# Gregor-Mendel-Institute/SNPmatch

Measured on AMD Instinct MI355X. Metric: accession×SNP comparisons/sec (whole node); achieved HBM GB/s vs peak, higher is better.
Workload: dtype f64

## Files before the change

snpmatch_amd/csrc/snpm_api_launch.hpp:

```cpp
struct FastGeom {
    bool packed;
    int wpb;
    int tile_rows = TILE_ROWS;
    int64_t n_wc, n_colblocks, n_parts, part_rows;
    int64_t n_epochs, n_slots, n_groups;
};

template <bool SKIP, bool GATHER>
int occupancy_of(int threads)
{
    int nb = 0;
    if (hipOccupancyMaxActiveBlocksPerMultiprocessor(&nb, k_fast<SKIP, GATHER>, threads, 0) != hipSuccess) nb = 0;
    return nb;
}

FastGeom fast_geom(snpm_ctx *ctx, int64_t n_acc, int64_t n, int occ_blocks_hint, bool packed, int tile_rows = TILE_ROWS,
                   int wpb_fixed = 0, int kernel_parts_mult = 1)
{
    FastGeom g;
    g.packed = packed;
    g.tile_rows = tile_rows;
    const int64_t span = (int64_t)WAVE * (packed ? 16 : 4);
    g.n_wc = std::max<int64_t>(1, (n_acc + span - 1) / span);
    if (wpb_fixed > 0) {
        g.wpb = (int)std::min<int64_t>(wpb_fixed, g.n_wc);
    } else if (g.n_wc <= 8) {
        g.wpb = (int)g.n_wc;
    } else {
        double best = -1.0;
        int best_w = 8;
        for (int w = 8; w >= 4; --w) {
            const int64_t blocks = (g.n_wc + w - 1) / w;
            const double active = (double)g.n_wc / (double)(blocks * w);
            const double balance = (w % 4 == 0) ? 1.0 : ((w % 2 == 0) ? 0.95 : 0.85);
            if (active * balance > best) { best = active * balance; best_w = w; }
        }
        g.wpb = best_w;
    }
    g.n_colblocks = (g.n_wc + g.wpb - 1) / g.wpb;
    int occ = occ_blocks_hint > 0 ? occ_blocks_hint : 2;
    const int64_t pitch_bytes = ((n_acc + 255) / 256) * 256;
    if (!packed && occ_blocks_hint > 0 && (g.wpb == 4 || g.wpb == 5) &&
        n * pitch_bytes >= (int64_t(32) << 30))
        occ = std::min(occ, std::max(3, 18 / g.wpb));
    if (!packed && occ_blocks_hint > 0 && g.wpb == 8 &&
        n * pitch_bytes >= (int64_t(4) << 30))
        occ = std::min(occ, 2);
    const int narrow_mult = (!packed && g.wpb == 1 && occ_blocks_hint > 0) ? 4 : 1;
    const int64_t n_tiles = std::max<int64_t>(1, (n + tile_rows - 1) / tile_rows);
    constexpr int64_t kPartMinTiles = 8;
    int kmult = 1;
    if (kernel_parts_mult > 1 && g.wpb != 5) {
        const int64_t base_parts = std::max<int64_t>(1, (int64_t)ctx->n_cu * occ * narrow_mult / g.n_colblocks);
        kmult = (int)std::max<int64_t>(1, std::min<int64_t>(kernel_parts_mult, n_tiles / (base_parts * kPartMinTiles)));
    }
    int64_t resident = (int64_t)ctx->n_cu * occ * narrow_mult * kmult;
    int64_t n_parts = std::max<int64_t>(1, resident / g.n_colblocks);
    n_parts = std::min(n_parts, n_tiles);
    if (ctx->debug_max_parts > 0) n_parts = std::min<int64_t>(n_parts, ctx->debug_max_parts);
    n_parts = std::min<int64_t>(n_parts, 65535);
    g.n_parts = n_parts;
    const int64_t tiles_per_part = (n_tiles + n_parts - 1) / n_parts;
    g.part_rows = tiles_per_part * tile_rows;
    g.n_epochs = std::max<int64_t>(1, (tiles_per_part + EPOCH_TILES - 1) / EPOCH_TILES);
    g.n_slots = g.n_epochs * g.n_parts;
    g.n_groups = (g.n_slots + REDUCE_GROUP - 1) / REDUCE_GROUP;
    return g;
}

template <bool SKIP, bool GATHER>
int launch_fast_t(snpm_query *q, const FastGeom &g)
{
    snpm_ctx *ctx = q->panel->ctx;
    snpm_panel *p = q->panel;
    dim3 grid((unsigned)g.n_colblocks, (unsigned)g.n_parts);
    dim3 block(WAVE * g.wpb);
    ProfScope ps(ctx, PK_FAST);
    if (g.tile_rows == LONG_TILE_ROWS)
        hipLaunchKernelGGL((k_fast<SKIP, GATHER, false, LONG_TILE_ROWS>), grid, block, 0, ctx->stream, p->d,
                           p->pitch, q->d_row_idx, q->row0, q->n, q->d_lut, (double *)ctx->ws_part_score.p, (uint32_t *)ctx->ws_part_miss.p,
                           p->ld, (const int64_t *)nullptr);
    else
        hipLaunchKernelGGL((k_fast<SKIP, GATHER>), grid, block, 0, ctx->stream, p->d, p->pitch, q->d_row_idx, q->row0,
                           q->n, q->d_lut, (double *)ctx->ws_part_score.p, (uint32_t *)ctx->ws_part_miss.p, p->ld,
                           (const int64_t *)nullptr, g.tile_rows < TILE_ROWS ? g.tile_rows : 0);
    HIPCHK(ctx, hipGetLastError());
    return SNPM_OK;
}

int launch_fast_b(snpm_query *q, const FastGeom &g, bool skip, bool gather)
{
    if (skip)
        return gather ? launch_fast_t<true, true>(q, g) : launch_fast_t<true, false>(q, g);
    return gather ? launch_fast_t<false, true>(q, g) : launch_fast_t<false, false>(q, g);
}

static int q4_waves_per_block(int64_t n_acc)
{
    const int64_t n_wc = (n_acc + 1023) / 1024;
    if (n_wc <= 8) return (int)n_wc;
    int best = 4;
    int64_t best_waves = (n_wc + 3) / 4 * 4;
    for (int w : {7, 8}) {
        const int64_t waves = (n_wc + w - 1) / w * w;
        if (waves <= best_waves) {
            best = w;
            best_waves = waves;
        }
    }
    return best;
}

static int q4_tile_rows(int wpb)
{
    return wpb >= 4 ? 64 : (wpb >= 2 ? 32 : 16);
}

template <bool SKIP, bool GATHER, int TR>
int launch_p16_t(snpm_query *q, const FastGeom &g, int *occ_out, int threads)
{
    snpm_ctx *ctx = q->panel->ctx;
    snpm_panel *p = q->panel;
    if (occ_out) {
        int nb = 0;
        if (hipOccupancyMaxActiveBlocksPerMultiprocessor(&nb, k_fast_packed_q4<SKIP, GATHER, false, TR>, threads, 0) != hipSuccess) nb = 0;
        *occ_out = nb;
        return SNPM_OK;
    }
    dim3 grid((unsigned)g.n_colblocks, (unsigned)g.n_parts);
    dim3 block(WAVE * g.wpb);
    ProfScope ps(ctx, PK_FAST);
    hipLaunchKernelGGL((k_fast_packed_q4<SKIP, GATHER, false, TR>), grid, block, 0, ctx->stream, p->d, p->kpitch, q->d_row_idx,
                       q->row0, q->n, q->d_lut, (double *)ctx->ws_part_score.p, (uint32_t *)ctx->ws_part_miss.p, p->ld, p->n_acc,
                       p->desc);
    HIPCHK(ctx, hipGetLastError());
    return SNPM_OK;
}

int launch_p16(snpm_query *q, const FastGeom &g, bool skip, bool gather, int *occ_out, int threads)
{
    const int tr = q4_tile_rows(threads / WAVE);
#define P16_CASE(S, G)                                                                              \
    if (skip == S && gather == G) {                                                                 \
        if (tr == 16) return launch_p16_t<S, G, 16>(q, g, occ_out, threads);                        \
        if (tr == 32) return launch_p16_t<S, G, 32>(q, g, occ_out, threads);                        \
        return launch_p16_t<S, G, 64>(q, g, occ_out, threads);                                      \
    }
    P16_CASE(false, false) P16_CASE(false, true) P16_CASE(true, false) P16_CASE(true, true)
#undef P16_CASE
    return SNPM_ERR_STATE;
}

template <bool SKIP, bool GATHER>
int launch_bits_t(snpm_query *q, const FastGeom &g, int *occ_out, int threads)
{
    snpm_ctx *ctx = q->panel->ctx;
    snpm_panel *p = q->panel;
    if (occ_out) {
        int nb = 0;
        if (hipOccupancyMaxActiveBlocksPerMultiprocessor(&nb, k_fast_bits<SKIP, GATHER>, threads, 0) != hipSuccess) nb = 0;
        *occ_out = nb;
        return SNPM_OK;
    }
    ProfScope ps(ctx, PK_FAST);
    hipLaunchKernelGGL((k_fast_bits<SKIP, GATHER>), dim3((unsigned)g.n_parts, (unsigned)g.n_colblocks), dim3(WAVE * g.wpb), 0,
                       ctx->stream, p->d, p->kpitch, q->d_row_idx, q->row0, q->n, (const uint8_t *)q->d_wbits,
                       (double *)ctx->ws_part_score.p, (uint32_t *)ctx->ws_part_miss.p, p->ld, p->n_acc, p->desc);
    HIPCHK(ctx, hipGetLastError());
    return SNPM_OK;
}

int launch_bits(snpm_query *q, const FastGeom &g, bool skip, bool gather, int *occ_out, int threads)
{
#define BITS_CASE(S, G) if (skip == S && gather == G) return launch_bits_t<S, G>(q, g, occ_out, threads)
    BITS_CASE(false, false); BITS_CASE(false, true); BITS_CASE(true, false); BITS_CASE(true, true);
#undef BITS_CASE
    return SNPM_ERR_STATE;
}

int occ_b(bool skip, bool gather, int threads)
{
    if (skip) return gather ? occupancy_of<true, true>(threads) : occupancy_of<true, false>(threads);
    return gather ? occupancy_of<false, true>(threads) : occupancy_of<false, false>(threads);
}

int ensure_lut(snpm_query *q, int skip)
{
    snpm_ctx *ctx = q->panel->ctx;
    if (q->lut_skip == skip) return SNPM_OK;
    if (q->n > 0) {
        ProfScope ps(ctx, PK_LUT);
        const int thr = 256;
        hipLaunchKernelGGL(k_build_lut, dim3((unsigned)((q->n + thr - 1) / thr)), dim3(thr), 0, ctx->stream, q->d_w,
                           q->d_lut, q->n, skip, (int *)nullptr);
        HIPCHK(ctx, hipGetLastError());
    }
    q->lut_skip = skip;
    return SNPM_OK;
}
```

snpmatch_amd/csrc/snpm_api_seg.hpp:

```cpp
struct SegJob {
    snpm_panel *p = nullptr;
    const int64_t *d_row_idx = nullptr;
    int64_t row0 = 0, n_total = 0;
    const double *d_w = nullptr, *d_lut = nullptr;
    const int64_t *seg_off = nullptr;
    int64_t n_seg = 0;
    int64_t chunk = 1000;
    int skip = 0;
    bool certify = true;
    double *d_score = nullptr;
    int64_t *d_ninfo = nullptr;
    int64_t ldo = 0;
    int64_t kmax = 1;
    int cap = 0;
    const int64_t *d_seg_off = nullptr;
};

constexpr int SEG_PAIR_CAP = 32768;

int *seg_pair_count(snpm_ctx *ctx) { return (int *)ctx->ws_pairs.p; }
int32_t *seg_pairs(snpm_ctx *ctx) { return (int32_t *)((char *)ctx->ws_pairs.p + 16); }

static int launch_q4_seg(snpm_ctx *ctx, const SegJob &j, dim3 grid, dim3 block, int64_t n_parts, const int64_t *d_desc)
{
    snpm_panel *p = j.p;
    const bool gather = j.d_row_idx != nullptr;
    ProfScope ps(ctx, PK_FAST);
    const int tr = q4_tile_rows((int)(block.x / WAVE));
#define LAUNCH_SEG_TR(S, G, TR)                                                                                   \
    hipLaunchKernelGGL((k_fast_packed_q4<S, G, true, TR>), grid, block, 0, ctx->stream, p->d, p->kpitch, j.d_row_idx, j.row0, \
                       n_parts, j.d_lut, (double *)ctx->ws_part_score.p, (uint32_t *)ctx->ws_part_miss.p, p->ld, p->n_acc, p->desc, d_desc)
#define LAUNCH_SEG(S, G)                                                                                          \
    do {                                                                                                          \
        if (tr == 16) LAUNCH_SEG_TR(S, G, 16);                                                                    \
        else if (tr == 32) LAUNCH_SEG_TR(S, G, 32);                                                               \
        else LAUNCH_SEG_TR(S, G, 64);                                                                             \
    } while (0)
    if (j.skip) {
        if (gather) LAUNCH_SEG(true, true); else LAUNCH_SEG(true, false);
    } else {
        if (gather) LAUNCH_SEG(false, true); else LAUNCH_SEG(false, false);
    }
#undef LAUNCH_SEG_TR
#undef LAUNCH_SEG
    HIPCHK(ctx, hipGetLastError());
    return SNPM_OK;
}

static int launch_fast_seg(snpm_ctx *ctx, const SegJob &j, dim3 grid, dim3 block, int64_t n_parts, const int64_t *d_desc)
{
    snpm_panel *p = j.p;
    const bool gather = j.d_row_idx != nullptr;
    ProfScope ps(ctx, PK_FAST);
#define LAUNCH_SEG(S, G)                                                                                          \
    hipLaunchKernelGGL((k_fast<S, G, true>), grid, block, 0, ctx->stream, p->d, p->pitch, j.d_row_idx, j.row0,    \
                       n_parts, j.d_lut, (double *)ctx->ws_part_score.p, (uint32_t *)ctx->ws_part_miss.p, p->ld, d_desc)
    if (j.skip) {
        if (gather) LAUNCH_SEG(true, true); else LAUNCH_SEG(true, false);
    } else {
        if (gather) LAUNCH_SEG(false, true); else LAUNCH_SEG(false, false);
    }
#undef LAUNCH_SEG
    HIPCHK(ctx, hipGetLastError());
    return SNPM_OK;
}

struct SegPlan {
    FastGeom g0;
    int64_t n_parts = 0, tiles_per_part = 0;
    std::vector<int64_t> slot0;
    const int64_t *d_slot0 = nullptr, *d_desc = nullptr;
};

static int seg_plan(snpm_ctx *ctx, SegJob &j, SegPlan &pl)
{
    snpm_panel *p = j.p;
    const int64_t n_seg = j.n_seg;
    const bool q4 = p->packed != 0;
    pl.g0 = q4 ? fast_geom(ctx, p->n_acc, TILE_ROWS, 2, true, TILE_ROWS, q4_waves_per_block(p->n_acc))
               : fast_geom(ctx, p->n_acc, TILE_ROWS, 2, false, TILE_ROWS);
    int64_t total_tiles = 0, kmax = 1;
    for (int64_t s = 0; s < n_seg; ++s) {
        const int64_t len = j.seg_off[s + 1] - j.seg_off[s];
        total_tiles += (len + TILE_ROWS - 1) / TILE_ROWS;
        kmax = std::max<int64_t>(kmax, (len + j.chunk - 1) / j.chunk);
    }
    const int per_cu = q4 ? 8 : 32;
    const int64_t want_blocks = std::max<int64_t>(1, std::min<int64_t>((int64_t)ctx->n_cu * per_cu / std::max<int64_t>(1, pl.g0.n_colblocks),
                                                                       std::max<int64_t>((int64_t)ctx->n_cu, 256 * n_seg)));
    pl.tiles_per_part = std::max<int64_t>(2, std::min<int64_t>(EPOCH_TILES, (total_tiles + want_blocks - 1) / want_blocks));
    const int64_t max_parts = total_tiles / pl.tiles_per_part + n_seg + 1;
    const size_t words = 2 * ((size_t)n_seg + 1) + 3 * (size_t)max_parts;
    if (ctx->h_desc_cap < words * sizeof(int64_t)) {
        HIPCHK(ctx, hipStreamSynchronize(ctx->stream));
        if (ctx->h_desc) (void)hipHostFree(ctx->h_desc);
        ctx->h_desc = nullptr;
        ctx->h_desc_cap = 0;
        HIPCHK(ctx, hipHostMalloc((void **)&ctx->h_desc, std::max<size_t>(words * sizeof(int64_t), 1 << 16), hipHostMallocDefault));
        ctx->h_desc_cap = std::max<size_t>(words * sizeof(int64_t), 1 << 16);
    } else {
        HIPCHK(ctx, hipStreamSynchronize(ctx->stream));
    }
    int64_t *h = ctx->h_desc;
    memcpy(h, j.seg_off, ((size_t)n_seg + 1) * sizeof(int64_t));
    const size_t o_slot0 = (size_t)n_seg + 1, o_desc = 2 * ((size_t)n_seg + 1);
    pl.slot0.assign((size_t)n_seg + 1, 0);
    int64_t n_parts = 0;
    size_t w = o_desc;
    for (int64_t s = 0; s < n_seg; ++s) {
        pl.slot0[(size_t)s] = n_parts;
        const int64_t r0 = j.seg_off[s], r1 = j.seg_off[s + 1];
        for (int64_t r = r0; r < r1; r += pl.tiles_per_part * TILE_ROWS) {
            h[w++] = r;
            h[w++] = std::min<int64_t>(r1, r + pl.tiles_per_part * TILE_ROWS);
            h[w++] = n_parts++;
        }
    }
    pl.slot0[(size_t)n_seg] = n_parts;
    memcpy(h + o_slot0, pl.slot0.data(), ((size_t)n_seg + 1) * sizeof(int64_t));
    pl.n_parts = n_parts;
    int rc = ensure(ctx, ctx->ws_seg_desc, w * sizeof(int64_t));
    if (rc) return rc;
    HIPCHK(ctx, hipMemcpyAsync(ctx->ws_seg_desc.p, h, w * sizeof(int64_t), hipMemcpyHostToDevice, ctx->stream));
    j.d_seg_off = (const int64_t *)ctx->ws_seg_desc.p;
    pl.d_slot0 = j.d_seg_off + o_slot0;
    pl.d_desc = j.d_seg_off + o_desc;
    j.kmax = kmax;
    j.cap = (int)std::max<int64_t>(64, std::min<int64_t>(SEG_PAIR_CAP, (int64_t(8) << 20) / kmax));
    rc = ensure(ctx, ctx->ws_part_score, (size_t)std::max<int64_t>(n_parts, 1) * p->ld * sizeof(double));
    if (rc) return rc;
    rc = ensure(ctx, ctx->ws_part_miss, (size_t)std::max<int64_t>(n_parts, 1) * p->ld * sizeof(uint32_t));
    if (rc) return rc;
    rc = ensure(ctx, ctx->ws_pairs, 16 + (size_t)SEG_PAIR_CAP * 2 * sizeof(int32_t));
    if (rc) return rc;
    HIPCHK(ctx, hipMemsetAsync(seg_pair_count(ctx), 0, sizeof(int), ctx->stream));
    if (j.certify) {
        rc = ensure(ctx, ctx->ws_eseg, (size_t)std::max<int64_t>(n_seg, 1) * sizeof(double));
        if (rc) return rc;
        rc = ensure(ctx, ctx->ws_pair_sums, (size_t)j.cap * (size_t)kmax * sizeof(double));
        if (rc) return rc;
    }
    return SNPM_OK;
}

static int seg_launch(snpm_ctx *ctx, const SegJob &j, const SegPlan &pl, int64_t s0, int64_t s1)
{
    snpm_panel *p = j.p;
    if (s1 <= s0) return SNPM_OK;
    int rc;
    if (j.certify) {
        const int64_t seg_parts = (j.kmax * j.chunk) / (pl.tiles_per_part * TILE_ROWS) + 2;
        const int npart = (int)((j.kmax + 3) / 4);
        rc = ensure(ctx, ctx->ws_epart, (size_t)(s1 - s0) * (size_t)npart * 3 * sizeof(double));
        if (rc) return rc;
        hipLaunchKernelGGL(k_eseg_part, dim3((unsigned)npart, (unsigned)(s1 - s0)), dim3(256), 0, ctx->stream, j.d_w,
                           j.d_seg_off, j.chunk, s0, npart, (double *)ctx->ws_epart.p);
        hipLaunchKernelGGL(k_eseg_finish, dim3((unsigned)(s1 - s0)), dim3(256), 0, ctx->stream,
                           (const double *)ctx->ws_epart.p, j.d_seg_off, j.chunk,
                           pl.tiles_per_part * TILE_ROWS + seg_parts + 2, s0, npart, (double *)ctx->ws_eseg.p);
        HIPCHK(ctx, hipGetLastError());
    }
    const int64_t p0 = pl.slot0[(size_t)s0], p1 = pl.slot0[(size_t)s1];
    if (p1 > p0) {
        const int64_t np = p1 - p0;
        const unsigned gy = (unsigned)std::min<int64_t>(np, 65535);
        const unsigned gz = (unsigned)((np + gy - 1) / gy);
        dim3 grid((unsigned)pl.g0.n_colblocks, gy, gz), block(WAVE * pl.g0.wpb);
        const int64_t *desc = pl.d_desc + 3 * p0;
        rc = p->packed ? launch_q4_seg(ctx, j, grid, block, np, desc) : launch_fast_seg(ctx, j, grid, block, np, desc);
        if (rc) return rc;
    }
    ProfScope ps(ctx, PK_REDUCE);
    const int thr = 64;
    hipLaunchKernelGGL(k_reduce_seg, dim3((unsigned)((p->n_acc + thr - 1) / thr), (unsigned)(s1 - s0)), dim3(thr), 0, ctx->stream,
                       (const double *)ctx->ws_part_score.p, (const uint32_t *)ctx->ws_part_miss.p, pl.d_slot0, j.d_seg_off,
                       p->ld, p->n_acc, j.d_score, j.d_ninfo, j.ldo,
                       j.certify ? (const double *)ctx->ws_eseg.p : (const double *)nullptr, ctx->debug_reeval,
                       seg_pairs(ctx), seg_pair_count(ctx), j.cap, s0);
    HIPCHK(ctx, hipGetLastError());
    return SNPM_OK;
}

static int seg_finish(snpm_ctx *ctx, const SegJob &j)
{
    snpm_panel *p = j.p;
    if (!j.certify || j.n_seg == 0) return SNPM_OK;
    const bool gather = j.d_row_idx != nullptr;
    if (single_accession(p)) {
        ProfScope ps(ctx, PK_STRICT);
        int rc = launch_strict_single(ctx, p, j.d_row_idx, j.row0, j.d_w, j.skip, j.d_seg_off, j.chunk, j.n_total, 0, j.n_seg,
                                      (const int32_t *)seg_pairs(ctx), (const int *)seg_pair_count(ctx), j.cap, 0, j.kmax,
                                      dim3((unsigned)std::min<int64_t>(std::max<int64_t>(j.kmax, 1), 1024), (unsigned)std::min(j.cap, 256)),
                                      (double *)ctx->ws_pair_sums.p, nullptr, 0);
        if (rc) return rc;
    } else {
        ProfScope ps(ctx, PK_STRICT);
        dim3 grid((unsigned)std::min<int64_t>(std::max<int64_t>(j.kmax, 1), 256), (unsigned)std::min(j.cap, 128));
#define LAUNCH_PAIRS(S, G)                                                                                        \
    hipLaunchKernelGGL((k_strict_pairs<S, G>), grid, dim3(WAVE), 0, ctx->stream, p->d, p->kpitch, p->desc, j.d_row_idx,     \
                       j.row0, j.d_w, j.d_seg_off, j.chunk, (const int32_t *)seg_pairs(ctx), (const int *)seg_pair_count(ctx), \
                       j.cap, j.kmax, (double *)ctx->ws_pair_sums.p)
        if (j.skip) {
            if (gather) LAUNCH_PAIRS(true, true); else LAUNCH_PAIRS(true, false);
        } else {
            if (gather) LAUNCH_PAIRS(false, true); else LAUNCH_PAIRS(false, false);
        }
#undef LAUNCH_PAIRS
        HIPCHK(ctx, hipGetLastError());
    }
    ProfScope ps(ctx, PK_SCAN);
    hipLaunchKernelGGL(k_scan_pairs, dim3((unsigned)std::min(j.cap, 1024)), dim3(64), 0, ctx->stream, (const double *)ctx->ws_pair_sums.p,
                       j.d_seg_off, j.chunk, (const int32_t *)seg_pairs(ctx), (const int *)seg_pair_count(ctx), j.cap, j.kmax,
                       j.d_score, j.ldo);
    HIPCHK(ctx, hipGetLastError());
    return SNPM_OK;
}

static int run_segmented(snpm_ctx *ctx, SegJob &j)
{
    if (j.n_seg == 0) return SNPM_OK;
    SegPlan pl;
    int rc = seg_plan(ctx, j, pl);
    if (!rc) rc = seg_launch(ctx, j, pl, 0, j.n_seg);
    if (!rc) rc = seg_finish(ctx, j);
    return rc;
}

static int ensure_stage(snpm_ctx *ctx)
{
    for (int i = 0; i < 2; ++i) {
        if (!ctx->stage[i]) {
            hipError_t e = hipHostMalloc(&ctx->stage[i], snpm_ctx::kStageBytes, hipHostMallocDefault);
            if (e != hipSuccess) return set_err(ctx, SNPM_ERR_OOM, "hipHostMalloc staging failed: %s", hipGetErrorString(e));
            HIPCHK(ctx, hipEventCreateWithFlags(&ctx->stage_done[i], hipEventDisableTiming));
        }
    }
    return SNPM_OK;
}

void parallel_copy(snpm_ctx *ctx, int8_t *dst, const int8_t *src, size_t n);

static int stage_bytes(snpm_ctx *ctx, void *d_dst, const void *h_src, size_t nbytes, bool src_pinned)
{
    if (nbytes == 0) return SNPM_OK;
    if (src_pinned) {
        HIPCHK(ctx, hipMemcpyAsync(d_dst, h_src, nbytes, hipMemcpyHostToDevice, ctx->copy_stream));
        return SNPM_OK;
    }
    for (size_t o = 0; o < nbytes; o += snpm_ctx::kStageBytes) {
        const size_t piece = std::min(snpm_ctx::kStageBytes, nbytes - o);
        const int which = ctx->stage_which;
        ctx->stage_which ^= 1;
        if (ctx->stage_busy[which]) {
            HIPCHK(ctx, hipEventSynchronize(ctx->stage_done[which]));
            ctx->stage_busy[which] = false;
        }
        parallel_copy(ctx, (int8_t *)ctx->stage[which], (const int8_t *)h_src + o, piece);
        HIPCHK(ctx, hipMemcpyAsync((char *)d_dst + o, ctx->stage[which], piece, hipMemcpyHostToDevice, ctx->copy_stream));
        HIPCHK(ctx, hipEventRecord(ctx->stage_done[which], ctx->copy_stream));
        ctx->stage_busy[which] = true;
    }
    return SNPM_OK;
}

static int stage_rows32(snpm_ctx *ctx, int32_t *d_dst, const int64_t *h_src, int64_t n)
{
    if (n == 0) return SNPM_OK;
    const int which = ctx->stage_which;
    ctx->stage_which ^= 1;
    if (ctx->stage_busy[which]) {
        HIPCHK(ctx, hipEventSynchronize(ctx->stage_done[which]));
        ctx->stage_busy[which] = false;
    }
    int32_t *slab = (int32_t *)ctx->stage[which];
    const int nthreads = (int)std::min<int64_t>(ctx->stage_threads, std::max<int64_t>(1, n >> 18));
    auto narrow = [=](int64_t a, int64_t b) {
        for (int64_t i = a; i < b; ++i) {
            const int64_t v = h_src[i];
            slab[i] = (v >= 0 && v <= 0x7fffffff) ? (int32_t)v : -1;
        }
    };
    if (nthreads <= 1) {
        narrow(0, n);
    } else {
        std::vector<std::thread> pool;
        const int64_t per = (n + nthreads - 1) / nthreads;
        for (int t = 0; t < nthreads; ++t)
            if (t * per < n) pool.emplace_back(narrow, t * per, std::min<int64_t>(n, (t + 1) * per));
        for (auto &th : pool) th.join();
    }
    HIPCHK(ctx, hipMemcpyAsync(d_dst, slab, (size_t)n * sizeof(int32_t), hipMemcpyHostToDevice, ctx->copy_stream));
    HIPCHK(ctx, hipEventRecord(ctx->stage_done[which], ctx->copy_stream));
    ctx->stage_busy[which] = true;
    return SNPM_OK;
}

static bool host_pointer_is_pinned(const void *ptr)
{
    hipPointerAttribute_t attr;
    if (hipPointerGetAttributes(&attr, ptr) != hipSuccess) {
        (void)hipGetLastError();
        return false;
    }
    return attr.type == hipMemoryTypeHost;
}

struct HostFetch {
    snpm_ctx *ctx;
    struct Item { void *dst; const void *src; size_t bytes; };
    Item items[8];
    int n_items = 0;
    size_t used = 0, cap = 0;
    explicit HostFetch(snpm_ctx *c) : ctx(c) {}
    int reserve(size_t total)
    {
        cap = 0;
        if (total == 0 || total > (size_t(256) << 20)) return ensure_pinned(ctx, 256);
        int rc = ensure_pinned(ctx, 256 + total);
        if (!rc) cap = total;
        return rc;
    }
    int add(void *host_dst, const void *dev_src, size_t bytes)
    {
        if (!host_dst || bytes == 0) return SNPM_OK;
        if (n_items < 8 && bytes <= (size_t(1) << 20) && used + bytes <= cap && !host_pointer_is_pinned(host_dst)) {
            char *slab = (char *)ctx->h_pinned + 256 + used;
            HIPCHK(ctx, hipMemcpyAsync(slab, dev_src, bytes, hipMemcpyDeviceToHost, ctx->stream));
            items[n_items++] = Item{host_dst, slab, bytes};
            used += (bytes + 63) & ~size_t(63);
        } else {
            HIPCHK(ctx, hipMemcpyAsync(host_dst, dev_src, bytes, hipMemcpyDeviceToHost, ctx->stream));
        }
        return SNPM_OK;
    }
    void finish()
    {
        for (int i = 0; i < n_items; ++i) parallel_copy(ctx, (int8_t *)items[i].dst, (const int8_t *)items[i].src, items[i].bytes);
        n_items = 0;
        used = 0;
    }
};

int read_count(snpm_query *q, int64_t *out)
{
    snpm_ctx *ctx = q->panel->ctx;
    *out = 0;
    if (!q->count_valid) return SNPM_OK;
    int rc = ensure_pinned(ctx, 64);
    if (rc) return rc;
    HIPCHK(ctx, hipMemcpyAsync(ctx->h_pinned, q->cert_count(), sizeof(int), hipMemcpyDeviceToHost, ctx->stream));
    HIPCHK(ctx, hipStreamSynchronize(ctx->stream));
    *out = *(const int *)ctx->h_pinned;
    return SNPM_OK;
}

int upload_seg_off(snpm_ctx *ctx, const std::vector<int64_t> &off)
{
    int rc = ensure(ctx, ctx->ws_seg_off, off.size() * sizeof(int64_t));
    if (rc) return rc;
    HIPCHK(ctx, hipMemcpyAsync(ctx->ws_seg_off.p, off.data(), off.size() * sizeof(int64_t), hipMemcpyHostToDevice,
                               ctx->stream));
    HIPCHK(ctx, hipStreamSynchronize(ctx->stream));
    return SNPM_OK;
}
```

snpmatch_amd/csrc/snpm_api_strict.hpp:

```cpp
static inline bool single_accession(const snpm_panel *p) { return p->n_acc_total == 1; }

static int launch_strict_single(snpm_ctx *ctx, const snpm_panel *p, const int64_t *d_row_idx, int64_t row0, const double *d_w,
                                int skip, const int64_t *seg_off, int64_t chunk, int64_t n, int64_t seg0, int64_t n_seg,
                                const int32_t *pairs, const int *count, int cap, int tier, int64_t kmax, dim3 grid,
                                double *out_score, uint32_t *out_miss, int64_t ld)
{
    const bool gather = d_row_idx != nullptr;
#define LAUNCH_SINGLE(S, G)                                                                                          \
    hipLaunchKernelGGL((k_strict_single<S, G>), grid, dim3(SINGLE_THREADS), 0, ctx->stream, p->d, p->kpitch, p->desc,  \
                       d_row_idx, row0, d_w, seg_off, chunk, n, seg0, n_seg, pairs, count, cap, tier, kmax, out_score,  \
                       out_miss, ld)
    if (skip) {
        if (gather) LAUNCH_SINGLE(true, true); else LAUNCH_SINGLE(true, false);
    } else {
        if (gather) LAUNCH_SINGLE(false, true); else LAUNCH_SINGLE(false, false);
    }
#undef LAUNCH_SINGLE
    HIPCHK(ctx, hipGetLastError());
    return SNPM_OK;
}

int launch_strict_dense(snpm_query *q, int skip, const int64_t *d_seg_off, int64_t chunk, int64_t seg0, int64_t n_seg,
                        const int *gate)
{
    snpm_ctx *ctx = q->panel->ctx;
    snpm_panel *p = q->panel;
    const int64_t ncols = p->n_acc, ld = p->ld;
    const bool gather = q->d_row_idx != nullptr;
    const int64_t *seg_off = d_seg_off ? d_seg_off + seg0 : nullptr;
    if (n_seg == 0) return SNPM_OK;
    if (single_accession(p)) {
        ProfScope ps(ctx, PK_STRICT);
        return launch_strict_single(ctx, p, q->d_row_idx, q->row0, q->d_w, skip, seg_off, chunk, q->n, seg0, n_seg, nullptr, gate,
                                    REEVAL_CAP, gate ? 2 : 0, 0, dim3((unsigned)std::min<int64_t>(n_seg, 65535)),
                                    (double *)ctx->ws_seg_score.p, (uint32_t *)ctx->ws_seg_miss.p, ld);
    }
    const int64_t lanes = (ncols + 3) / 4;
    const int t4 = lanes >= 256 ? 256 : (lanes > 64 ? 128 : 64);
    dim3 grid4((unsigned)(gate ? std::min<int64_t>(n_seg, 2048) : n_seg), (unsigned)((lanes + t4 - 1) / t4));
    ProfScope ps(ctx, PK_STRICT);
#define LAUNCH_STRICT4(S, G)                                                                                     \
    do {                                                                                                     \
        if (p->packed)                                                                                       \
            hipLaunchKernelGGL((k_strict4<S, G, true>), grid4, dim3(t4), 0, ctx->stream, p->d, p->kpitch, q->d_row_idx, q->row0, \
                               q->d_w, seg_off, chunk, q->n, seg0, n_seg, ncols, (double *)ctx->ws_seg_score.p,  \
                               (uint32_t *)ctx->ws_seg_miss.p, ld, (const int *)nullptr, gate, REEVAL_CAP, p->desc); \
        else                                                                                                 \
            hipLaunchKernelGGL((k_strict4<S, G, false>), grid4, dim3(t4), 0, ctx->stream, p->d, p->pitch, q->d_row_idx, q->row0, \
                               q->d_w, seg_off, chunk, q->n, seg0, n_seg, ncols, (double *)ctx->ws_seg_score.p,  \
                               (uint32_t *)ctx->ws_seg_miss.p, ld, (const int *)p->d_other, gate, REEVAL_CAP);   \
    } while (0)
    if (skip) {
        if (gather) LAUNCH_STRICT4(true, true); else LAUNCH_STRICT4(true, false);
    } else {
        if (gather) LAUNCH_STRICT4(false, true); else LAUNCH_STRICT4(false, false);
    }
#undef LAUNCH_STRICT4
    HIPCHK(ctx, hipGetLastError());
    return SNPM_OK;
}

constexpr size_t kStrictGroupBytes = size_t(512) << 20;

int run_strict_chain(snpm_query *q, int skip, int64_t chunk, const int *gate, const double *carry_score,
                     const int64_t *carry_ninfo, double *dst_score, int64_t *dst_ninfo)
{
    snpm_ctx *ctx = q->panel->ctx;
    snpm_panel *p = q->panel;
    const int64_t n_seg = (q->n + chunk - 1) / chunk;
    const int64_t per_seg = p->ld * (int64_t)(sizeof(double) + sizeof(uint32_t));
    const int64_t group = std::max<int64_t>(1, std::min<int64_t>(std::max<int64_t>(n_seg, 1), (int64_t)kStrictGroupBytes / per_seg));
    int rc = ensure(ctx, ctx->ws_seg_score, (size_t)group * p->ld * sizeof(double));
    if (rc) return rc;
    rc = ensure(ctx, ctx->ws_seg_miss, (size_t)group * p->ld * sizeof(uint32_t));
    if (rc) return rc;
    const int thr = 256;
    const unsigned cb = (unsigned)((p->n_acc + thr - 1) / thr);
    bool first = true;
    for (int64_t g0 = 0; g0 < n_seg || first; g0 += group) {
        const int64_t ns = std::max<int64_t>(0, std::min<int64_t>(group, n_seg - g0));
        rc = launch_strict_dense(q, skip, nullptr, chunk, g0, ns, gate);
        if (rc) return rc;
        const int64_t rows = std::min<int64_t>(q->n, (g0 + ns) * chunk) - std::min<int64_t>(q->n, g0 * chunk);
        ProfScope ps(ctx, PK_SCAN);
        hipLaunchKernelGGL(k_scan, dim3(cb), dim3(thr), 0, ctx->stream, (const double *)ctx->ws_seg_score.p,
                           (const uint32_t *)ctx->ws_seg_miss.p, rows, ns, p->ld, p->n_acc, dst_score, dst_ninfo,
                           first ? carry_score : (const double *)dst_score, first ? carry_ninfo : (const int64_t *)dst_ninfo,
                           gate, REEVAL_CAP);
        HIPCHK(ctx, hipGetLastError());
        first = false;
    }
    return SNPM_OK;
}

struct OnceTail {
    const int64_t *d_ninfo = nullptr;
    int64_t n_acc = 0;
    int want_lik = 0;
    unsigned *state = nullptr;
    double *lik_tmp = nullptr;
    int64_t *out = nullptr;
};

int run_strict_sparse(snpm_query *q, int skip, int64_t chunk, const int32_t *d_cols, const int *d_ncols, const double *carry,
                      const int64_t *d_seg_off = nullptr, int64_t n_seg_explicit = 0, double *patch_score = nullptr,
                      const OnceTail *tail = nullptr)
{
    snpm_ctx *ctx = q->panel->ctx;
    snpm_panel *p = q->panel;
    const int64_t n_seg = d_seg_off ? n_seg_explicit : (q->n + chunk - 1) / chunk;
    const int64_t ld = REEVAL_CAP;
    int rc = ensure(ctx, ctx->ws_seg_score, (size_t)std::max<int64_t>(n_seg, 1) * ld * sizeof(double));
    if (rc) return rc;
    rc = ensure(ctx, ctx->ws_seg_miss, (size_t)std::max<int64_t>(n_seg, 1) * ld * sizeof(uint32_t));
    if (rc) return rc;
    rc = ensure(ctx, ctx->ws_tmp_score, (size_t)ld * sizeof(double));
    if (rc) return rc;
    const bool gather = q->d_row_idx != nullptr;
    const int64_t total = n_seg * ld;
    if (total > 0) {
        dim3 sgrid((unsigned)std::min<int64_t>((total + 255) / 256, (int64_t)ctx->n_cu * 8));
        const bool use_T = !q->transient_panel && q->n >= ctx->acc_major_min_rows && p->dT_state == 1;
        ProfScope ps(ctx, PK_STRICT);
        if (single_accession(p)) {
            q->reeval_path = 2;
            rc = launch_strict_single(ctx, p, q->d_row_idx, q->row0, q->d_w, skip, d_seg_off, chunk, q->n, 0, n_seg, nullptr, d_ncols,
                                      REEVAL_CAP, 1, 0, dim3((unsigned)std::min<int64_t>(n_seg, 65535)),
                                      (double *)ctx->ws_seg_score.p, (uint32_t *)ctx->ws_seg_miss.p, ld);
            if (rc) return rc;
        } else if (use_T) {
            q->reeval_path = 1;
#define LAUNCH_SPARSE_T(S, G)                                                                                      \
    hipLaunchKernelGGL((k_strict_sparse_T<S, G>), sgrid, dim3(256), 0, ctx->stream, p->dT, p->pitchT, q->d_row_idx, \
                       q->row0, q->d_w, d_seg_off, chunk, q->n, n_seg, d_cols, d_ncols, REEVAL_CAP, \
                       (double *)ctx->ws_seg_score.p, (uint32_t *)ctx->ws_seg_miss.p, ld)
            if (skip) {
                if (gather) LAUNCH_SPARSE_T(true, true); else LAUNCH_SPARSE_T(true, false);
            } else {
                if (gather) LAUNCH_SPARSE_T(false, true); else LAUNCH_SPARSE_T(false, false);
            }
#undef LAUNCH_SPARSE_T
        } else {
            q->reeval_path = 2;
#define LAUNCH_SPARSE(S, G)                                                                                        \
    hipLaunchKernelGGL((k_strict_sparse<S, G>), sgrid, dim3(256), 0, ctx->stream, p->d, p->kpitch, p->desc, q->d_row_idx, \
                       q->row0, q->d_w, d_seg_off, chunk, q->n, n_seg, d_cols, d_ncols, REEVAL_CAP, \
                       (double *)ctx->ws_seg_score.p, (uint32_t *)ctx->ws_seg_miss.p, ld)
            if (skip) {
                if (gather) LAUNCH_SPARSE(true, true); else LAUNCH_SPARSE(true, false);
            } else {
                if (gather) LAUNCH_SPARSE(false, true); else LAUNCH_SPARSE(false, false);
            }
#undef LAUNCH_SPARSE
        }
        HIPCHK(ctx, hipGetLastError());
    }
    ProfScope ps(ctx, PK_SCAN);
    if (tail)
        hipLaunchKernelGGL(k_once_tail, dim3(1), dim3(256), 0, ctx->stream, (const double *)ctx->ws_seg_score.p, n_seg, ld, d_ncols,
                           REEVAL_CAP, (double *)ctx->ws_tmp_score.p, d_cols, patch_score, tail->d_ninfo, tail->n_acc, tail->want_lik,
                           tail->state, tail->lik_tmp, tail->out);
    else
        hipLaunchKernelGGL(k_scan_few, dim3(1), dim3(256), 0, ctx->stream, (const double *)ctx->ws_seg_score.p, n_seg, ld,
                           d_ncols, REEVAL_CAP, (double *)ctx->ws_tmp_score.p, carry, d_cols, patch_score);
    HIPCHK(ctx, hipGetLastError());
    return SNPM_OK;
}
```

snpmatch_amd/csrc/snpm_k_fast.hpp:

```cpp
#pragma once

namespace snpm {
template <int NDW, bool SKIP, int U>
__device__ __forceinline__ void fast_row(const uint32_t (&x)[NDW], uint32_t group_base, uint32_t roff4,
                                         double (&acc)[NDW * 4], uint32_t (&miss8)[NDW])
{
#ifdef SNPM_FAST_PATTERN_ONLY
#pragma unroll
    for (int k = 0; k < NDW; ++k) miss8[k] ^= x[k];
    (void)group_base; (void)roff4; (void)acc;
    return;
#endif
    double w[NDW * 4];
#pragma unroll
    for (int k = 0; k < NDW; ++k) {
        const uint32_t tix = ((x[k] << 3) & 0x18181818u) | roff4;
        if (SKIP)
            miss8[k] += ((x[k] >> 7) | ((x[k] >> 1) & ~x[k])) & 0x01010101u;
        else
            miss8[k] += (x[k] >> 7) & 0x01010101u;
#pragma unroll
        for (int j = 0; j < 4; ++j) {
            const uint32_t addr = __builtin_amdgcn_perm(tix, group_base, 0x0c0c0100u | (uint32_t)(4 + j));
            lds_cdouble *ptr = (lds_cdouble *)(uintptr_t)addr;
            w[4 * k + j] = ptr[U * 4];
        }
    }
#pragma unroll
    for (int e = 0; e < NDW * 4; ++e) acc[e] += w[e];
}

__device__ __forceinline__ void load_row(const int8_t *p, uint32_t (&x)[1])
{
    x[0] = __builtin_nontemporal_load(reinterpret_cast<const uint32_t *>(p));
}

#define SCORE_ROW(U, X, GROUP_BASE, ROFF4, ROFF) fast_row<NDW, SKIP, U>((X), (GROUP_BASE), (ROFF4), acc, miss8)

template <bool SKIP, bool GATHER, bool SEG = false, int TR = TILE_ROWS>
__global__ void __launch_bounds__(WAVE *MAX_WAVES_PER_BLOCK, SNPM_FAST_MIN_WAVES)
k_fast(const int8_t *__restrict__ db, int64_t pitch, const int64_t *__restrict__ row_idx, int64_t row0, int64_t n,
       const double *__restrict__ lut, double *__restrict__ out_score, uint32_t *__restrict__ out_miss, int64_t ld,
       const int64_t *__restrict__ part_desc = nullptr, int tile_rows_rt = 0)
{
    constexpr int BPL = 4;
    constexpr int NDW = BPL / 4;
    constexpr int EPL = BPL;
    constexpr int G = GATHER ? SNPM_FAST_G_GATHER : SNPM_FAST_G;
    __shared__ __attribute__((aligned(256))) double s_lut[2][TR * 4];
    const int TRR = (tile_rows_rt > 0 && tile_rows_rt <= TR) ? tile_rows_rt : TR;

    const int tid = threadIdx.x;
    const int nthr = blockDim.x;
    const int64_t byte0 = ((int64_t)blockIdx.x * nthr + tid) * BPL;
    const int64_t col0 = byte0;
    const bool lane_on = byte0 < pitch && col0 < ld;
    const int64_t p = SEG ? (int64_t)blockIdx.y + (int64_t)gridDim.y * blockIdx.z : (int64_t)blockIdx.y;
    if (SEG && p >= n) return;
    const int64_t rbase = SEG ? part_desc[3 * p] : 0;
    const int64_t rend = SEG ? part_desc[3 * p + 1] : n;
    const int64_t P = SEG ? 1 : (int64_t)gridDim.y;
    const int64_t T0 = SEG ? 0 : p;
    const int64_t slot0 = SEG ? part_desc[3 * p + 2] : p;
    const int64_t slot_stride = SEG ? 1 : (int64_t)gridDim.y;
    const int64_t n_tiles_total = (rend - rbase + TRR - 1) / TRR;

    double acc[EPL];
    uint32_t miss16[NDW * 2];
    uint32_t miss8[NDW];
#pragma unroll
    for (int i = 0; i < EPL; ++i) acc[i] = 0.0;
#pragma unroll
    for (int i = 0; i < NDW * 2; ++i) miss16[i] = 0;
#pragma unroll
    for (int i = 0; i < NDW; ++i) miss8[i] = 0;

    const uint32_t lane_off = lane_on ? (uint32_t)byte0 : 0u;
    auto row_ptr = [&](int64_t rr) -> const int8_t * {
        const int64_t prow = GATHER ? row_idx[rr] : (row0 + rr);
        const int8_t *rowbase = db + prow * pitch;
        uint32_t off = lane_off;
        asm volatile("" : "+v"(off));
        return rowbase + off;
    };

    auto store_partials = [&](int64_t epoch) {
        if (lane_on) {
            double *os = out_score + (slot0 + epoch * slot_stride) * ld + col0;
            uint32_t *om = out_miss + (slot0 + epoch * slot_stride) * ld + col0;
#pragma unroll
            for (int i = 0; i < EPL; i += 2) *reinterpret_cast<double2 *>(os + i) = make_double2(acc[i], acc[i + 1]);
#pragma unroll
            for (int k = 0; k < NDW; ++k) {
                uint4 m;
                m.x = miss16[2 * k + 0] & 0xffffu;
                m.y = miss16[2 * k + 1] & 0xffffu;
                m.z = miss16[2 * k + 0] >> 16;
                m.w = miss16[2 * k + 1] >> 16;
                *reinterpret_cast<uint4 *>(om + 4 * k) = m;
            }
        }
#pragma unroll
        for (int i = 0; i < EPL; ++i) acc[i] = 0.0;
#pragma unroll
        for (int i = 0; i < NDW * 2; ++i) miss16[i] = 0;
    };
    int64_t last_epoch = 0;

    if (T0 < n_tiles_total) {
        {
            const int64_t tr0 = rbase + T0 * TRR;
            const int rows2 = 2 * (int)((rend - tr0 < TRR) ? (rend - tr0) : TRR);
            const double2 *src = reinterpret_cast<const double2 *>(lut + 4 * tr0);
            double2 *dst = reinterpret_cast<double2 *>(&s_lut[0][0]);
            for (int i = tid; i < rows2; i += nthr) dst[i] = src[i];
        }
        uint32_t xa[G][NDW], xb[G][NDW];
#pragma unroll
        for (int u = 0; u < G; ++u) load_row(row_ptr(rbase + T0 * TRR + u), xa[u]);
        __syncthreads();

        int buf = 0;
        int tiles_in_epoch = 0;
        int64_t epoch = 0;
        for (int64_t T = T0; T < n_tiles_total; T += P, buf ^= 1) {
            if (tiles_in_epoch == EPOCH_TILES) {
                store_partials(epoch);
                ++epoch;
                tiles_in_epoch = 0;
            }
            ++tiles_in_epoch;
            const int64_t tr0 = rbase + T * TRR;
            const int rows = (int)((rend - tr0 < TRR) ? (rend - tr0) : TRR);
            const bool more = (T + P < n_tiles_total);
            const int64_t ntr0 = more ? rbase + (T + P) * TRR : tr0;
            double2 pre0 = make_double2(0.0, 0.0);
            const bool staged = more && nthr >= TRR * 2;
            const int nrows2 = more ? 2 * (int)((rend - ntr0 < TRR) ? (rend - ntr0) : TRR) : 0;
#if !defined(SNPM_FAST_PATTERN_ONLY) || SNPM_FAST_PATTERN_ONLY != 2
            if (staged && tid < nrows2) pre0 = reinterpret_cast<const double2 *>(lut + 4 * ntr0)[tid];
#endif

            const uint32_t lds_base =
                (uint32_t)(uintptr_t)(__attribute__((address_space(3))) double *)(&s_lut[buf][0]);
            const int full_groups = rows / G;
#define SCORE_GROUP(X, GI)                                                                  \
    do {                                                                                    \
        const uint32_t goff_ = (uint32_t)(GI) * (uint32_t)(G * LUT_ROW_BYTES);              \
        const uint32_t gbase_ = lds_base + (goff_ & ~255u);                                 \
        const uint32_t roff_ = goff_ & 255u;                                                \
        const uint32_t roff4_ = roff_ * 0x01010101u;                                        \
        SCORE_ROW(0, (X)[0], gbase_, roff4_, roff_);                                        \
        SCORE_ROW(1, (X)[1], gbase_, roff4_, roff_);                                        \
        if constexpr (G > 2) {                                                              \
            SCORE_ROW(2, (X)[G > 2 ? 2 : 0], gbase_, roff4_, roff_);                        \
            SCORE_ROW(3, (X)[G > 2 ? 3 : 0], gbase_, roff4_, roff_);                        \
        }                                                                                   \
        if constexpr (G > 4) {                                                              \
            SCORE_ROW(4, (X)[G > 4 ? 4 : 0], gbase_, roff4_, roff_);                        \
            SCORE_ROW(5, (X)[G > 4 ? 5 : 0], gbase_, roff4_, roff_);                        \
            SCORE_ROW(6, (X)[G > 4 ? 6 : 0], gbase_, roff4_, roff_);                        \
            SCORE_ROW(7, (X)[G > 4 ? 7 : 0], gbase_, roff4_, roff_);                        \
        }                                                                                   \
    } while (0)
            int g = 0;
            for (; g + 2 <= full_groups; g += 2) {
                const int64_t rnext = tr0 + (int64_t)(g + 1) * G;
                const int64_t rafter = (g + 2 < TRR / G) ? rnext + G : ntr0;
#pragma unroll
                for (int u = 0; u < G; ++u) load_row(row_ptr(rnext + u), xb[u]);
                SCORE_GROUP(xa, g);
#pragma unroll
                for (int u = 0; u < G; ++u) load_row(row_ptr(rafter + u), xa[u]);
                SCORE_GROUP(xb, g + 1);
            }
            if (g < full_groups) {
                SCORE_GROUP(xa, g);
            }
#undef SCORE_GROUP
            for (int r = full_groups * G; r < rows; ++r) {
                uint32_t x[NDW];
                load_row(row_ptr(tr0 + r), x);
                const uint32_t group_base = lds_base + (uint32_t)(r >> 3) * 256u;
                const uint32_t roff4 = (uint32_t)(r & 7) * 0x20202020u;
                SCORE_ROW(0, x, group_base, roff4, (uint32_t)(r & 7) * 32u);
            }
#pragma unroll
            for (int k = 0; k < NDW; ++k) {
                miss16[2 * k + 0] += miss8[k] & 0x00ff00ffu;
                miss16[2 * k + 1] += (miss8[k] >> 8) & 0x00ff00ffu;
                miss8[k] = 0;
            }
#if !defined(SNPM_FAST_PATTERN_ONLY) || SNPM_FAST_PATTERN_ONLY != 2
            if (more) {
                double2 *dst = reinterpret_cast<double2 *>(&s_lut[buf ^ 1][0]);
                if (staged) {
                    if (tid < TRR * 2) dst[tid] = pre0;
                } else {
                    const double2 *src = reinterpret_cast<const double2 *>(lut + 4 * ntr0);
                    for (int i = tid; i < nrows2; i += nthr) dst[i] = src[i];
                }
            }
            __syncthreads();
#endif
        }
        last_epoch = epoch;
    }
    store_partials(last_epoch);
}

#undef SCORE_ROW

}
```

Measured before the change: 6145 billion.

## Redirect padding-lane loads in fast kernel to real data and resize sparse launches

```diff
diff --git a/snpmatch_amd/csrc/snpm_api_launch.hpp b/snpmatch_amd/csrc/snpm_api_launch.hpp
--- a/snpmatch_amd/csrc/snpm_api_launch.hpp
+++ b/snpmatch_amd/csrc/snpm_api_launch.hpp
@@ -68,7 +68,12 @@
     return g;
 }
 
-template <bool SKIP, bool GATHER>
+static inline bool fast_has_pad_line(const snpm_panel *p)
+{
+    return p->pitch - (p->n_acc + 127) / 128 * 128 >= 128;
+}
+
+template <bool SKIP, bool GATHER, bool PAD>
 int launch_fast_t(snpm_query *q, const FastGeom &g)
 {
     snpm_ctx *ctx = q->panel->ctx;
@@ -77,12 +82,12 @@
     dim3 block(WAVE * g.wpb);
     ProfScope ps(ctx, PK_FAST);
     if (g.tile_rows == LONG_TILE_ROWS)
-        hipLaunchKernelGGL((k_fast<SKIP, GATHER, false, LONG_TILE_ROWS>), grid, block, 0, ctx->stream, p->d,
+        hipLaunchKernelGGL((k_fast<SKIP, GATHER, false, LONG_TILE_ROWS, PAD>), grid, block, 0, ctx->stream, p->d,
                            p->pitch, q->d_row_idx, q->row0, q->n, q->d_lut, (double *)ctx->ws_part_score.p, (uint32_t *)ctx->ws_part_miss.p,
-                           p->ld, (const int64_t *)nullptr);
+                           p->ld, p->n_acc, (const int64_t *)nullptr);
     else
-        hipLaunchKernelGGL((k_fast<SKIP, GATHER>), grid, block, 0, ctx->stream, p->d, p->pitch, q->d_row_idx, q->row0,
-                           q->n, q->d_lut, (double *)ctx->ws_part_score.p, (uint32_t *)ctx->ws_part_miss.p, p->ld,
+        hipLaunchKernelGGL((k_fast<SKIP, GATHER, false, TILE_ROWS, PAD>), grid, block, 0, ctx->stream, p->d, p->pitch, q->d_row_idx, q->row0,
+                           q->n, q->d_lut, (double *)ctx->ws_part_score.p, (uint32_t *)ctx->ws_part_miss.p, p->ld, p->n_acc,
                            (const int64_t *)nullptr, g.tile_rows < TILE_ROWS ? g.tile_rows : 0);
     HIPCHK(ctx, hipGetLastError());
     return SNPM_OK;
@@ -90,9 +95,14 @@
 
 int launch_fast_b(snpm_query *q, const FastGeom &g, bool skip, bool gather)
 {
+    if (fast_has_pad_line(q->panel)) {
+        if (skip)
+            return gather ? launch_fast_t<true, true, true>(q, g) : launch_fast_t<true, false, true>(q, g);
+        return gather ? launch_fast_t<false, true, true>(q, g) : launch_fast_t<false, false, true>(q, g);
+    }
     if (skip)
-        return gather ? launch_fast_t<true, true>(q, g) : launch_fast_t<true, false>(q, g);
-    return gather ? launch_fast_t<false, true>(q, g) : launch_fast_t<false, false>(q, g);
+        return gather ? launch_fast_t<true, true, false>(q, g) : launch_fast_t<true, false, false>(q, g);
+    return gather ? launch_fast_t<false, true, false>(q, g) : launch_fast_t<false, false, false>(q, g);
 }
 
 static int q4_waves_per_block(int64_t n_acc)
diff --git a/snpmatch_amd/csrc/snpm_api_seg.hpp b/snpmatch_amd/csrc/snpm_api_seg.hpp
--- a/snpmatch_amd/csrc/snpm_api_seg.hpp
+++ b/snpmatch_amd/csrc/snpm_api_seg.hpp
@@ -52,15 +52,21 @@
     snpm_panel *p = j.p;
     const bool gather = j.d_row_idx != nullptr;
     ProfScope ps(ctx, PK_FAST);
+#define LAUNCH_SEG_P(S, G, PAD)                                                                                   \
+    hipLaunchKernelGGL((k_fast<S, G, true, TILE_ROWS, PAD>), grid, block, 0, ctx->stream, p->d, p->pitch, j.d_row_idx, j.row0, \
+                       n_parts, j.d_lut, (double *)ctx->ws_part_score.p, (uint32_t *)ctx->ws_part_miss.p, p->ld, \
+                       p->n_acc, d_desc)
 #define LAUNCH_SEG(S, G)                                                                                          \
-    hipLaunchKernelGGL((k_fast<S, G, true>), grid, block, 0, ctx->stream, p->d, p->pitch, j.d_row_idx, j.row0,    \
-                       n_parts, j.d_lut, (double *)ctx->ws_part_score.p, (uint32_t *)ctx->ws_part_miss.p, p->ld, d_desc)
+    do {                                                                                                          \
+        if (fast_has_pad_line(p)) LAUNCH_SEG_P(S, G, true); else LAUNCH_SEG_P(S, G, false);                       \
+    } while (0)
     if (j.skip) {
         if (gather) LAUNCH_SEG(true, true); else LAUNCH_SEG(true, false);
     } else {
         if (gather) LAUNCH_SEG(false, true); else LAUNCH_SEG(false, false);
     }
 #undef LAUNCH_SEG
+#undef LAUNCH_SEG_P
     HIPCHK(ctx, hipGetLastError());
     return SNPM_OK;
 }
diff --git a/snpmatch_amd/csrc/snpm_api_strict.hpp b/snpmatch_amd/csrc/snpm_api_strict.hpp
--- a/snpmatch_amd/csrc/snpm_api_strict.hpp
+++ b/snpmatch_amd/csrc/snpm_api_strict.hpp
@@ -119,7 +119,8 @@
     const bool gather = q->d_row_idx != nullptr;
     const int64_t total = n_seg * ld;
     if (total > 0) {
-        dim3 sgrid((unsigned)std::min<int64_t>((total + 255) / 256, (int64_t)ctx->n_cu * 8));
+        const int sthr = total > (int64_t)256 * ctx->n_cu ? WAVE : 256;
+        dim3 sgrid((unsigned)std::min<int64_t>((total + sthr - 1) / sthr, (int64_t)ctx->n_cu * (2048 / sthr)));
         const bool use_T = !q->transient_panel && q->n >= ctx->acc_major_min_rows && p->dT_state == 1;
         ProfScope ps(ctx, PK_STRICT);
         if (single_accession(p)) {
@@ -131,7 +132,7 @@
         } else if (use_T) {
             q->reeval_path = 1;
 #define LAUNCH_SPARSE_T(S, G)                                                                                      \
-    hipLaunchKernelGGL((k_strict_sparse_T<S, G>), sgrid, dim3(256), 0, ctx->stream, p->dT, p->pitchT, q->d_row_idx, \
+    hipLaunchKernelGGL((k_strict_sparse_T<S, G>), sgrid, dim3(sthr), 0, ctx->stream, p->dT, p->pitchT, q->d_row_idx, \
                        q->row0, q->d_w, d_seg_off, chunk, q->n, n_seg, d_cols, d_ncols, REEVAL_CAP, \
                        (double *)ctx->ws_seg_score.p, (uint32_t *)ctx->ws_seg_miss.p, ld)
             if (skip) {
@@ -143,7 +144,7 @@
         } else {
             q->reeval_path = 2;
 #define LAUNCH_SPARSE(S, G)                                                                                        \
-    hipLaunchKernelGGL((k_strict_sparse<S, G>), sgrid, dim3(256), 0, ctx->stream, p->d, p->kpitch, p->desc, q->d_row_idx, \
+    hipLaunchKernelGGL((k_strict_sparse<S, G>), sgrid, dim3(sthr), 0, ctx->stream, p->d, p->kpitch, p->desc, q->d_row_idx, \
                        q->row0, q->d_w, d_seg_off, chunk, q->n, n_seg, d_cols, d_ncols, REEVAL_CAP, \
                        (double *)ctx->ws_seg_score.p, (uint32_t *)ctx->ws_seg_miss.p, ld)
             if (skip) {
diff --git a/snpmatch_amd/csrc/snpm_k_fast.hpp b/snpmatch_amd/csrc/snpm_k_fast.hpp
--- a/snpmatch_amd/csrc/snpm_k_fast.hpp
+++ b/snpmatch_amd/csrc/snpm_k_fast.hpp
@@ -37,11 +37,11 @@
 
 #define SCORE_ROW(U, X, GROUP_BASE, ROFF4, ROFF) fast_row<NDW, SKIP, U>((X), (GROUP_BASE), (ROFF4), acc, miss8)
 
-template <bool SKIP, bool GATHER, bool SEG = false, int TR = TILE_ROWS>
+template <bool SKIP, bool GATHER, bool SEG = false, int TR = TILE_ROWS, bool PAD = false>
 __global__ void __launch_bounds__(WAVE *MAX_WAVES_PER_BLOCK, SNPM_FAST_MIN_WAVES)
 k_fast(const int8_t *__restrict__ db, int64_t pitch, const int64_t *__restrict__ row_idx, int64_t row0, int64_t n,
        const double *__restrict__ lut, double *__restrict__ out_score, uint32_t *__restrict__ out_miss, int64_t ld,
-       const int64_t *__restrict__ part_desc = nullptr, int tile_rows_rt = 0)
+       int64_t n_acc, const int64_t *__restrict__ part_desc = nullptr, int tile_rows_rt = 0)
 {
     constexpr int BPL = 4;
     constexpr int NDW = BPL / 4;
@@ -55,6 +55,8 @@
     const int64_t byte0 = ((int64_t)blockIdx.x * nthr + tid) * BPL;
     const int64_t col0 = byte0;
     const bool lane_on = byte0 < pitch && col0 < ld;
+    const bool pad_lane = PAD && lane_on && byte0 >= (n_acc + 127) / 128 * 128;
+    const uint32_t pad18 = pad_lane ? 0x18181818u : 0u;
     const int64_t p = SEG ? (int64_t)blockIdx.y + (int64_t)gridDim.y * blockIdx.z : (int64_t)blockIdx.y;
     if (SEG && p >= n) return;
     const int64_t rbase = SEG ? part_desc[3 * p] : 0;
@@ -75,7 +77,7 @@
 #pragma unroll
     for (int i = 0; i < NDW; ++i) miss8[i] = 0;
 
-    const uint32_t lane_off = lane_on ? (uint32_t)byte0 : 0u;
+    const uint32_t lane_off = !lane_on ? 0u : (pad_lane ? (uint32_t)((n_acc - 1) & ~(int64_t)3) : (uint32_t)byte0);
     auto row_ptr = [&](int64_t rr) -> const int8_t * {
         const int64_t prow = GATHER ? row_idx[rr] : (row0 + rr);
         const int8_t *rowbase = db + prow * pitch;
@@ -149,7 +151,7 @@
         const uint32_t goff_ = (uint32_t)(GI) * (uint32_t)(G * LUT_ROW_BYTES);              \
         const uint32_t gbase_ = lds_base + (goff_ & ~255u);                                 \
         const uint32_t roff_ = goff_ & 255u;                                                \
-        const uint32_t roff4_ = roff_ * 0x01010101u;                                        \
+        const uint32_t roff4_ = (roff_ * 0x01010101u) | pad18;                              \
         SCORE_ROW(0, (X)[0], gbase_, roff4_, roff_);                                        \
         SCORE_ROW(1, (X)[1], gbase_, roff4_, roff_);                                        \
         if constexpr (G > 2) {                                                              \
@@ -182,11 +184,12 @@
                 uint32_t x[NDW];
                 load_row(row_ptr(tr0 + r), x);
                 const uint32_t group_base = lds_base + (uint32_t)(r >> 3) * 256u;
-                const uint32_t roff4 = (uint32_t)(r & 7) * 0x20202020u;
+                const uint32_t roff4 = ((uint32_t)(r & 7) * 0x20202020u) | pad18;
                 SCORE_ROW(0, x, group_base, roff4, (uint32_t)(r & 7) * 32u);
             }
 #pragma unroll
             for (int k = 0; k < NDW; ++k) {
+                if (pad_lane) miss8[k] = (uint32_t)rows * 0x01010101u;
                 miss16[2 * k + 0] += miss8[k] & 0x00ff00ffu;
                 miss16[2 * k + 1] += (miss8[k] >> 8) & 0x00ff00ffu;
                 miss8[k] = 0;
```

Measured after the change: 6257 billion, median of 6. 1.02x the previous value.
